# microsoft/hyperspace

Measured on AMD Instinct MI355X. Metric: index-build GB/s + indexed filter/join query latency (s), 1/2/4/8 MI355X, higher is better.
Workload: dtype int64/fp64 columnar; 1 GPU; model=covering-index(key,val) build + filter + co-bucketed join, num_buckets=200, parallelism=bucket-parallel dp1, RCCL all-to-all exchange, device=cuda

## Files before the change

### hyperspace_amd/csrc/binding.cpp

```cpp

#include <torch/extension.h>

#include <c10/hip/HIPStream.h>

#include <algorithm>
#include <string>
#include <tuple>
#include <vector>

#include "bucket_writer.h"
#include "kernels/kernels.h"

namespace {

hipStream_t current_stream() {
  return c10::hip::getCurrentHIPStream().stream();
}

void check_cuda(const torch::Tensor& t, const char* name) {
  TORCH_CHECK(t.is_cuda(), name, " must be a device tensor");
  TORCH_CHECK(t.is_contiguous(), name, " must be contiguous");
}

int normalize_dtype_code(torch::ScalarType t) {
// ... 500 lines not shown
                     ((uint32_t)d[pos + 3] << 24);
      pos += 4;
      TORCH_CHECK(pos + (int64_t)len <= end, "byte-array page ", p,
                  ": value overruns page");
      op[vi++] = (int32_t)written;
      memcpy(bp + written, d + pos, len);
      written += len;
      pos += len;
    }
  }
  op[vi] = (int32_t)written;
  return {offs, out.narrow(0, 0, written)};
}

void host_memcpy(torch::Tensor dst, int64_t off, py::buffer src) {
  TORCH_CHECK(!dst.is_cuda() && dst.scalar_type() == torch::kUInt8,
              "dst must be a cpu u8 tensor");
  py::buffer_info info = src.request();
  int64_t n = (int64_t)info.size * (int64_t)info.itemsize;
  TORCH_CHECK(off >= 0 && off + n <= dst.numel(),
              "host_memcpy out of range");
  uint8_t* d = dst.data_ptr<uint8_t>() + off;
  const void* s = info.ptr;
  {
    py::gil_scoped_release rel;
    memcpy(d, s, (size_t)n);
  }
}

std::vector<torch::Tensor> parse_rle_runs(torch::Tensor bytes,
                                           int64_t start, int64_t end,
                                           int64_t bit_width,
                                           int64_t num_values) {
  TORCH_CHECK(!bytes.is_cuda() && bytes.scalar_type() == torch::kUInt8,
              "bytes must be a cpu u8 tensor");
  const uint8_t* d = bytes.data_ptr<uint8_t>();
  std::vector<int64_t> kind, out_off, len, bitoff, value;
  int64_t pos = start, out = 0;
  int64_t bw_bytes = (bit_width + 7) / 8;
  while (out < num_values && pos < end) {
    uint64_t h = 0;
    int shift = 0;
    while (true) {
      TORCH_CHECK(pos < end, "rle: truncated varint");
      uint8_t b = d[pos++];
      h |= (uint64_t)(b & 0x7F) << shift;
      if (!(b & 0x80)) break;
      shift += 7;
    }
    if (h & 1) {
      int64_t groups = (int64_t)(h >> 1);
      int64_t count = groups * 8;
      if (count > num_values - out) count = num_values - out;
      kind.push_back(1);
      out_off.push_back(out);
      len.push_back(count);
      bitoff.push_back(pos * 8);
      value.push_back(0);
      pos += groups * bit_width;
      out += count;
    } else {
      int64_t run = (int64_t)(h >> 1);
      if (run > num_values - out) run = num_values - out;
      int64_t v = 0;
      for (int64_t i = 0; i < bw_bytes; i++) {
        TORCH_CHECK(pos < end, "rle: truncated repeat value");
        v |= (int64_t)d[pos++] << (8 * i);
      }
      kind.push_back(0);
      out_off.push_back(out);
      len.push_back(run);
      bitoff.push_back(0);
      value.push_back(v);
      out += run;
    }
  }
  TORCH_CHECK(out == num_values, "rle: produced ", out, " of ",
              num_values, " values");
  auto opts = torch::dtype(torch::kInt64);
  auto mk = [&](std::vector<int64_t>& v) {
    return torch::tensor(v, opts);
  };
  return {mk(kind), mk(out_off), mk(len), mk(bitoff), mk(value)};
}

torch::Tensor rle_decode(torch::Tensor src_u8_dev, torch::Tensor kind,
                         torch::Tensor out_off, torch::Tensor len,
                         torch::Tensor bitoff, torch::Tensor value,
                         int64_t bit_width, int64_t n_out) {
  check_cuda(src_u8_dev, "src");
  TORCH_CHECK(bit_width >= 0 && bit_width <= 32,
              "rle_decode: bit_width must be in 0..32, got ", bit_width);
  auto dev = src_u8_dev.device();
  auto k = kind.to(dev), o = out_off.to(dev), l = len.to(dev),
       b = bitoff.to(dev), v = value.to(dev);
  auto out = torch::empty({n_out},
                          torch::dtype(torch::kInt32).device(dev));
  hsk::rle_decode_indices(src_u8_dev.data_ptr<uint8_t>(),
                          k.data_ptr<int64_t>(), o.data_ptr<int64_t>(),
                          l.data_ptr<int64_t>(), b.data_ptr<int64_t>(),
                          v.data_ptr<int64_t>(), kind.numel(),
                          (int)bit_width,
                          (uint32_t*)out.data_ptr<int32_t>(), n_out,
                          current_stream());
  return out;
}

void copy_unaligned(torch::Tensor src_u8, int64_t src_off,
                    torch::Tensor dst, int64_t dst_byte_off,
                    int64_t nbytes) {
  TORCH_CHECK(src_u8.is_cuda() && dst.is_cuda(), "device tensors required");
  TORCH_CHECK(src_u8.scalar_type() == torch::kUInt8, "src must be u8");
  TORCH_CHECK(src_off + nbytes + 4 <= src_u8.numel(),
              "src buffer must extend 4 bytes past the payload");
  TORCH_CHECK(dst_byte_off % 4 == 0 && nbytes % 4 == 0, "4B granularity");
  hsk::copy_unaligned(src_u8.data_ptr<uint8_t>(), src_off,
                      (uint8_t*)dst.data_ptr(), dst_byte_off, nbytes,
                      current_stream());
}

torch::Tensor gather_rows(torch::Tensor values, torch::Tensor idx) {
  check_cuda(values, "values");
  check_cuda(idx, "idx");
  TORCH_CHECK(idx.scalar_type() == torch::kInt64 ||
                  idx.scalar_type() == torch::kInt32,
              "idx must be int64 or int32");
  auto out = torch::empty({idx.numel()}, values.options());
  if (idx.scalar_type() == torch::kInt32)
    hsk::gather(values.data_ptr(), idx.data_ptr<int32_t>(), out.data_ptr(),
                idx.numel(), (int)values.element_size(), current_stream());
  else
    hsk::gather(values.data_ptr(), idx.data_ptr<int64_t>(), out.data_ptr(),
                idx.numel(), (int)values.element_size(), current_stream());
  return out;
}

int bit_length_u64(uint64_t v) { return v ? 64 - __builtin_clzll(v) : 0; }

py::object bucket_sort_perm(torch::Tensor key, torch::Tensor bucket_ids,
                            int64_t num_buckets) {
  check_cuda(key, "key");
  check_cuda(bucket_ids, "bucket_ids");
  TORCH_CHECK(bucket_ids.scalar_type() == torch::kInt32,
              "bucket_ids must be int32");
  TORCH_CHECK(num_buckets > 0 && num_buckets <= (int64_t)INT32_MAX,
              "bucket_sort_perm: num_buckets must be in 1..INT32_MAX, got ",
              num_buckets);
  int dtype = normalize_dtype_code(key.scalar_type());
  TORCH_CHECK(dtype != 2 && dtype != 3,
              "bucket_sort_perm: integer keys only");
  int64_t n = key.numel();
  TORCH_CHECK(bucket_ids.numel() == n, "bucket_ids length mismatch");
  if (n <= 1 || n > (int64_t)INT32_MAX) return py::none();
  auto dev = key.device();
  auto i64 = torch::dtype(torch::kInt64).device(dev);
  auto i32 = torch::dtype(torch::kInt32).device(dev);
  auto stream = current_stream();

  auto mm = torch::empty({2}, i64);
  hsk::key_minmax(key.data_ptr(), dtype, n,
                  (uint64_t*)mm.data_ptr<int64_t>(), stream);
  auto mm_host = mm.cpu();
  uint64_t kmin = (uint64_t)mm_host.data_ptr<int64_t>()[0];
  uint64_t range = (uint64_t)mm_host.data_ptr<int64_t>()[1] - kmin;
  int bbits = bit_length_u64((uint64_t)num_buckets - 1);
  int kbits = bit_length_u64(range);
  if (kbits + bbits > 64) return py::none();
  int shift = (kbits + 7) / 8 * 8;
  if (shift + bbits > 64) shift = 64 - bbits;
  uint64_t low_mask = kbits ? ~0ull >> (64 - kbits) : 0;
  uint64_t mask = low_mask;
  if (bbits) mask |= (~0ull >> (64 - bbits)) << shift;

  auto comp = torch::empty({n}, i64);
  auto tmp_comp = torch::empty({n}, i64);
  auto perm = torch::empty({n}, i32);
  auto tmp_perm = torch::empty({n}, i32);
  auto hist = torch::empty({hsk::radix_sort_hist_size(n)}, i32);
  hsk::compose_bucket_key(key.data_ptr(), dtype,
                          bucket_ids.data_ptr<int32_t>(), kmin, shift,
                          (uint64_t*)comp.data_ptr<int64_t>(), n, stream);
  if (hsk::radix_sort_index32((uint64_t*)comp.data_ptr<int64_t>(),
                              perm.data_ptr<int32_t>(),
                              (uint64_t*)tmp_comp.data_ptr<int64_t>(),
                              tmp_perm.data_ptr<int32_t>(),
                              (uint32_t*)hist.data_ptr<int32_t>(), mask, n,
                              stream)) {
    std::swap(comp, tmp_comp);
    std::swap(perm, tmp_perm);
  }
  auto sorted = (const uint64_t*)comp.data_ptr<int64_t>();
  auto seg = torch::empty({num_buckets + 1}, i64);
  hsk::bucket_seg_offsets(sorted, n, shift, (int32_t)num_buckets,
                          seg.data_ptr<int64_t>(), stream);
  auto sorted_key = torch::empty_like(key);
  hsk::restore_key(sorted, low_mask, kmin, dtype, sorted_key.data_ptr(), n,
                   stream);
  return py::make_tuple(perm, sorted_key, seg.cpu());
}

torch::Tensor aligned16(torch::Tensor t) {
  if (t.numel() > 0 && reinterpret_cast<uintptr_t>(t.data_ptr()) % 16 != 0)
    return t.clone();
  return t;
}

torch::Tensor group_offsets(std::vector<torch::Tensor> keys,
                            std::vector<torch::Tensor> masks) {
  TORCH_CHECK(!keys.empty() && keys.size() <= 8, "1..8 key columns");
  TORCH_CHECK(masks.empty() || masks.size() == keys.size(),
              "masks must be empty or parallel to keys");
  int64_t n = keys[0].numel();
  auto dev = keys[0].device();
  auto opts = torch::dtype(torch::kInt64).device(dev);
  if (n == 0) return torch::zeros({1}, opts);
  std::vector<torch::Tensor> held;
  const uint64_t* kptr[8] = {nullptr};
  const uint8_t* mptr[8] = {nullptr};
  for (size_t c = 0; c < keys.size(); ++c) {
    check_cuda(keys[c], "key");
    TORCH_CHECK(keys[c].scalar_type() == torch::kInt64,
                "keys must be normalized int64");
    TORCH_CHECK(keys[c].numel() == n, "key column length mismatch");
    held.push_back(aligned16(keys[c]));
    kptr[c] = (const uint64_t*)held.back().data_ptr<int64_t>();
    if (!masks.empty() && masks[c].numel() > 0) {
      check_cuda(masks[c], "mask");
      TORCH_CHECK(masks[c].numel() == n, "mask length mismatch");
      TORCH_CHECK(masks[c].scalar_type() == torch::kBool ||
                      masks[c].scalar_type() == torch::kUInt8,
                  "mask must be bool/uint8");
      held.push_back(aligned16(masks[c]));
      mptr[c] = (const uint8_t*)held.back().data_ptr();
    }
  }
  auto stream = current_stream();
  int64_t tile = hsk::group_tile_size();
  int64_t n_tiles = (n + tile - 1) / tile;
  auto tile_counts = torch::empty({n_tiles}, opts);
  hsk::group_offsets_count(kptr, mptr, (int)keys.size(), n,
                           tile_counts.data_ptr<int64_t>(), stream);
  auto tile_offsets = torch::empty({n_tiles}, opts);
  auto total = torch::empty({1}, opts);
  hsk::exclusive_scan_i64(tile_counts.data_ptr<int64_t>(),
                          tile_offsets.data_ptr<int64_t>(), n_tiles,
                          total.data_ptr<int64_t>(), stream);
  int64_t n_groups = total.cpu().item<int64_t>();
  auto out = torch::empty({n_groups + 1}, opts);
  hsk::group_offsets_emit(kptr, mptr, (int)keys.size(), n,
                          tile_offsets.data_ptr<int64_t>(),
                          total.data_ptr<int64_t>(), out.data_ptr<int64_t>(),
                          stream);
  return out;
}

std::vector<torch::Tensor> segmented_reduce(torch::Tensor values,
                                            torch::Tensor valid,
                                            torch::Tensor offsets,
                                            int64_t want) {
  check_cuda(values, "values");
  int dtype;
  switch (values.scalar_type()) {
    case torch::kInt64: dtype = 0; break;
    case torch::kInt32: dtype = 1; break;
    case torch::kFloat64: dtype = 2; break;
    case torch::kFloat32: dtype = 3; break;
    default:
      TORCH_CHECK(false, "segmented_reduce: values must be int32, int64, "
                         "float32 or float64");
  }
  bool is_float = dtype >= 2;
  auto dev = values.device();
  int64_t n = values.numel();
  auto off_d = offsets.to(dev, torch::kInt64).contiguous();
  TORCH_CHECK(off_d.numel() >= 1, "offsets must have n_groups + 1 entries");
  int64_t n_groups = off_d.numel() - 1;
  auto i64 = torch::dtype(torch::kInt64).device(dev);
  auto sum_opts = is_float ? torch::dtype(torch::kFloat64).device(dev) : i64;
  auto sums = torch::zeros({(want & 1) ? n_groups : 0}, sum_opts);
  auto mins = torch::zeros({(want & 2) ? n_groups : 0}, values.options());
  auto maxs = torch::zeros({(want & 4) ? n_groups : 0}, values.options());
  auto counts = torch::zeros({n_groups}, i64);
  if (n == 0 || n_groups == 0) return {sums, mins, maxs, counts};
  values = aligned16(values);
  const uint8_t* vptr = nullptr;
  if (valid.numel() > 0) {
    check_cuda(valid, "valid");
    TORCH_CHECK(valid.numel() == n, "valid length mismatch");
    TORCH_CHECK(valid.scalar_type() == torch::kBool ||
                    valid.scalar_type() == torch::kUInt8,
                "valid must be bool/uint8");
    valid = aligned16(valid);
    vptr = (const uint8_t*)valid.data_ptr();
  }
  int64_t tile = hsk::group_tile_size();
  int64_t n_tiles = (n + tile - 1) / tile;
  auto tile_groups = torch::empty({n_tiles + 1}, i64);
  auto partials =
      torch::empty({4 * hsk::segmented_reduce_num_blocks(n)}, i64);
  hsk::segmented_reduce(values.data_ptr(), dtype, vptr,
                        off_d.data_ptr<int64_t>(), n, n_groups,
                        (want & 1) ? sums.data_ptr() : nullptr,
                        (want & 2) ? mins.data_ptr() : nullptr,
                        (want & 4) ? maxs.data_ptr() : nullptr,
                        counts.data_ptr<int64_t>(),
                        tile_groups.data_ptr<int64_t>(),
                        partials.data_ptr<int64_t>(), current_stream());
  return {sums, mins, maxs, counts};
}

int64_t group_tile_size() { return hsk::group_tile_size(); }

torch::Tensor topk_rows(torch::Tensor keys, int64_t k, torch::Tensor valid,
                        bool keep_ties) {
  check_cuda(keys, "keys");
  TORCH_CHECK(keys.scalar_type() == torch::kInt64,
              "keys must be normalized int64");
  int64_t n = keys.numel();
  auto opts = torch::dtype(torch::kInt64).device(keys.device());
  if (n == 0 || k <= 0) return torch::empty({0}, opts);
  if (k > n) k = n;
  keys = aligned16(keys);
  const uint8_t* vptr = nullptr;
  if (valid.numel() > 0) {
    check_cuda(valid, "valid");
    TORCH_CHECK(valid.numel() == n, "valid length mismatch");
    TORCH_CHECK(valid.scalar_type() == torch::kBool ||
                    valid.scalar_type() == torch::kUInt8,
                "valid must be bool/uint8");
    valid = aligned16(valid);
    vptr = (const uint8_t*)valid.data_ptr();
  }
  auto stream = current_stream();
  auto scratch = torch::zeros({hsk::topk_scratch_size(n)}, opts);
  const uint64_t* kp = (const uint64_t*)keys.data_ptr<int64_t>();
  int64_t* d_total = hsk::topk_select(kp, vptr, n, k, keep_ties,
                                      scratch.data_ptr<int64_t>(), stream);
  int64_t idx = d_total - scratch.data_ptr<int64_t>();
  int64_t n_out = scratch.narrow(0, idx, 1).cpu().item<int64_t>();
  TORCH_CHECK(n_out >= 0 && n_out <= n, "topk_rows: bad output length");
  auto out = torch::empty({n_out}, opts);
  hsk::topk_emit(kp, vptr, n, scratch.data_ptr<int64_t>(),
                 out.data_ptr<int64_t>(), n_out, stream);
  return out;
}

int64_t topk_tile_size() { return hsk::topk_tile_size(); }

std::tuple<std::vector<int64_t>, std::vector<int64_t>, std::vector<int64_t>,
           std::vector<int64_t>>
write_bucket_files(std::vector<torch::Tensor> cols,
// ... 195 lines not shown
```

### hyperspace_amd/execution/scan_stream.py

```python

from __future__ import annotations

from concurrent.futures import ThreadPoolExecutor
from typing import Iterator, List, Optional, Tuple

import torch

from .columnar import ColumnBatch
from ..config import IndexConstants


class ScanStream:
    def __init__(self, files, columns: List[str], device,
                 lineage_tracker=None, group_bytes: int = 1 << 30,
                 reader=None):
        self.files = list(files)
        self.columns = list(columns)
        self.device = device
        self.tracker = lineage_tracker
        self.group_bytes = max(1, group_bytes)
        self.reader = reader

    @property
    def total_bytes(self) -> int:
        return sum(f.size for f in self.files)

    def file_groups(self) -> List[List]:
        groups: List[List] = []
        cur: List = []
        cur_bytes = 0
        for f in self.files:
            if cur and cur_bytes + f.size > self.group_bytes:
                groups.append(cur)
                cur = []
                cur_bytes = 0
            cur.append(f)
            cur_bytes += f.size
        if cur:
            groups.append(cur)
        return groups

    def _load_group(self, group) -> ColumnBatch:
        paths = [f.name for f in group]
        if self.reader is not None:
            batch, row_counts = self.reader(paths, self.columns or None,
                                            self.device)
        else:
            from ..sources.parquet_io import (read_files_batch,
                                              read_files_batch_device)
            if self.device.type == "cuda":
                batch, row_counts = read_files_batch_device(
                    paths, self.device, columns=self.columns or None)
            else:
                batch, row_counts = read_files_batch(
                    paths, columns=self.columns or None)
        if self.tracker is not None:
            fids = torch.tensor(
                [self.tracker.add_file(f.name, f.size, f.modifiedTime)
                 for f in group], dtype=torch.int64, device=batch.device)
            counts = torch.tensor(row_counts, dtype=torch.int64,
                                  device=batch.device)
            batch = batch.with_column(
                IndexConstants.DATA_FILE_NAME_ID_COLUMN,
                torch.repeat_interleave(fids, counts))
        return batch

    def batches(self) -> Iterator[ColumnBatch]:
        groups = self.file_groups()
        if not groups:
            return
        with ThreadPoolExecutor(max_workers=1) as prefetcher:
            fut = prefetcher.submit(self._load_group, groups[0])
            for i in range(len(groups)):
                batch = fut.result()
                if i + 1 < len(groups):
                    fut = prefetcher.submit(self._load_group,
                                            groups[i + 1])
                yield batch

    def materialize(self) -> ColumnBatch:
        parts = list(self.batches())
        if not parts:
            from ..execution.executor import _empty_batch
            from ..log.entry import Schema, SchemaField
            return ColumnBatch({})
        if len(parts) == 1:
            return parts[0]
        return ColumnBatch.concat(parts)
```

### hyperspace_amd/index/covering/index.py

```python

from __future__ import annotations

import contextlib
import os
from typing import Any, Dict, List, Optional, Tuple

import torch

from ..base import Index, IndexerContext
from ...config import IndexConstants
from ...exceptions import HyperspaceException
from ...log.entry import (Schema, register_derived_dataset,
                          COVERING_INDEX_TYPE)
from ... import ops
from ...execution.columnar import ColumnBatch, StringColumn
from ...sources.parquet_io import (bucket_file_name, write_batch_parquet,
                                   read_files_batch, bucket_id_of_file)


class CoveringIndex(Index):
    def __init__(self, indexed_columns: List[str],
                 included_columns: List[str], schema: Schema,
                 num_buckets: int, properties: Dict[str, str]):
        self.indexed_columns = list(indexed_columns)
        self.included_columns = list(included_columns)
        self.schema = schema
        self.num_buckets = num_buckets
        self._properties = dict(properties)

    @property
    def kind(self) -> str:
        return "CoveringIndex"

    @property
    def kind_abbr(self) -> str:
        return "CI"

    def indexed_columns_list(self) -> List[str]:
        return list(self.indexed_columns)

    def referenced_columns(self) -> List[str]:
        return self.indexed_columns + self.included_columns

    @property
    def can_handle_deleted_files(self) -> bool:
        return (self._properties.get(IndexConstants.LINEAGE_PROPERTY, "false")
                .lower() == "true")

    @property
    def has_lineage(self) -> bool:
        return self.can_handle_deleted_files

    def with_new_properties(self, props: Dict[str, str]) -> "CoveringIndex":
        return CoveringIndex(self.indexed_columns, self.included_columns,
                             self.schema, self.num_buckets, props)

    def to_json(self) -> Dict[str, Any]:
        return {
            "type": COVERING_INDEX_TYPE,
            "indexedColumns": self.indexed_columns,
            "includedColumns": self.included_columns,
            "schema": self.schema.to_json(),
            "numBuckets": self.num_buckets,
            "properties": self._properties,
        }

    @staticmethod
    def from_json(d: Dict[str, Any]) -> "CoveringIndex":
        return CoveringIndex(
            d["indexedColumns"], d["includedColumns"],
            Schema.from_json(d["schema"]), d["numBuckets"],
            d.get("properties", {}))

    def write(self, ctx: IndexerContext, index_data) -> List[str]:
        from ...execution.scan_stream import ScanStream
        os.makedirs(ctx.index_data_path, exist_ok=True)

        import torch.distributed as dist
        distributed = dist.is_available() and dist.is_initialized() and \
            dist.get_world_size() > 1
        task_id = dist.get_rank() if distributed else 0

        if isinstance(index_data, ScanStream):
            batches = index_data.batches()
            n_groups = len(index_data.file_groups())
        else:
            batches = iter([index_data])
            n_groups = 1

        if distributed:
            from ...parallel import dist_context as dc
            t = dc.collective_tensor([n_groups])
            dist.all_reduce(t, op=dist.ReduceOp.MAX)
            n_groups = int(t[0])
            written = self._write_distributed(ctx, batches, n_groups,
                                              task_id)
        else:
            written = []
            for g in range(n_groups):
                try:
                    batch = next(batches)
                except StopIteration:
                    batch = self._empty_batch(ctx)
                written.extend(self._write_group(ctx, batch, task_id))
        if n_groups > 1:
            ctx.built_for_cache = None
        return written

    def _bucket_ids(self, batch: ColumnBatch) -> torch.Tensor:
        from ...ops.string_hash import bucket_hash_keys
        keys = bucket_hash_keys(batch, self.indexed_columns)
        key_masks = [batch.mask(c) for c in self.indexed_columns]
        return ops.murmur3_bucket(
            keys, self.num_buckets,
            key_masks if any(m is not None for m in key_masks) else None)

    def _write_distributed(self, ctx, batches, n_groups: int,
                           task_id: int) -> List[str]:
        import torch.distributed as dist
        from ...parallel import dist_context as dc
        from ...parallel.exchange import BucketExchange
        n = self.num_buckets
        ex = BucketExchange(n)
        ctx.exchange_stats = ex
        chunk_bytes = int(ctx.session.conf.get(
            "spark.hyperspace.exchange.chunkBytes", 1 << 30))
        written: List[str] = []
        recv_acc: Dict[int, list] = {}

        def flush_group(g: int) -> None:
            parts = recv_acc.pop(g, [])
            parts = [(b, k) for b, k in parts if b.num_rows]
            if not parts:
                return
            if len(parts) == 1:
                rb, rbk = parts[0]
            else:
                rb = ColumnBatch.concat([p[0] for p in parts])
                rbk = torch.cat([p[1] for p in parts])
            batch, seg = sort_by_bucket_and_keys(
                rb, rbk, self.indexed_columns, n)
            out = write_bucketed(batch, seg, ctx.index_data_path, n,
                                 task_id)
            ctx.built_for_cache = (batch, seg, list(out))
            written.extend(out)

        prev = None
        for g in range(n_groups):
            try:
                batch = next(batches)
            except StopIteration:
                batch = self._empty_batch(ctx)
            local_chunks = 1
            if chunk_bytes > 0 and batch.num_rows:
                local_chunks = max(
                    1, -(-batch.nbytes() // chunk_bytes))
            t = dc.collective_tensor([local_chunks])
            dist.all_reduce(t, op=dist.ReduceOp.MAX)
            nchunks = int(t[0])
            rows = batch.num_rows
            for c in range(nchunks):
                lo = rows * c // nchunks
                hi = rows * (c + 1) // nchunks
                sub = batch.slice(lo, hi) if nchunks > 1 else batch
                pend = ex.start(sub, self._bucket_ids(sub))
                if prev is not None:
                    p, pg, plast = prev
                    recv_acc.setdefault(pg, []).append(ex.finish(p))
                    if plast:
                        flush_group(pg)
                prev = (pend, g, c == nchunks - 1)
        if prev is not None:
            p, pg, _ = prev
            recv_acc.setdefault(pg, []).append(ex.finish(p))
            flush_group(pg)
        return written

    def _write_group(self, ctx, batch: ColumnBatch,
                     task_id: int) -> List[str]:
        import time as _time
        timing = os.environ.get("HS_TIMING")
        n = self.num_buckets
        t0 = _time.perf_counter()
        bucket_ids = self._bucket_ids(batch)
        if batch.num_rows == 0:
            return []
        t1 = _time.perf_counter()

        pipeline = (batch.device.type == "cuda" and n >= 8
                    and batch.num_rows >= 1 << 22
                    and bool(os.environ.get("HS_PIPE_WRITE")))
        if not pipeline:
            batch, seg = sort_by_bucket_and_keys(
                batch, bucket_ids, self.indexed_columns, n)
            if timing:
                import torch as _torch
                if batch.device.type == "cuda":
                    _torch.cuda.synchronize()
            t2 = _time.perf_counter()
            out = write_bucketed(batch, seg, ctx.index_data_path, n,
                                 task_id)
            ctx.built_for_cache = (batch, seg, list(out))
            if timing:
                import sys as _sys
                print(f"[hs-timing] build group: hash {t1-t0:.3f}s "
                      f"sort {t2-t1:.3f}s write "
                      f"{_time.perf_counter()-t2:.3f}s",
                      file=_sys.stderr)
            return out

        import torch as _torch
        from concurrent.futures import ThreadPoolExecutor
        b64 = bucket_ids.to(_torch.int64)
        perm = ops.sort_perm(ops.normalize_key(b64))
        batch = batch.gather(perm)
        sorted_b = ops.gather_rows(b64, perm)
        seg = _bucket_seg_offsets(sorted_b, n)
        t2 = _time.perf_counter()

        nb_batches = min(8, n)
        bounds = [round(i * n / nb_batches) for i in range(nb_batches + 1)]
        pool = ThreadPoolExecutor(max_workers=2)
        futures = []
        pieces: List[ColumnBatch] = []
        for i in range(nb_batches):
            b_lo, b_hi = bounds[i], bounds[i + 1]
            r_lo, r_hi = int(seg[b_lo]), int(seg[b_hi])
            if r_hi <= r_lo:
                continue
            sub = batch.slice(r_lo, r_hi)
            sub_sorted, lseg = sort_by_bucket_and_keys(
                sub, sorted_b[r_lo:r_hi], self.indexed_columns, n)
            ev = _torch.cuda.Event()
            ev.record()
            pieces.append(sub_sorted)
            futures.append(pool.submit(
                write_bucketed, sub_sorted, lseg, ctx.index_data_path,
                n, task_id, ev))
        out = []
        for f in futures:
            out.extend(f.result())
        pool.shutdown()
        if timing:
            _torch.cuda.synchronize()
        t3 = _time.perf_counter()
        full = (ColumnBatch.concat(pieces) if len(pieces) > 1
                else pieces[0]) if pieces else batch
        ctx.built_for_cache = (full, seg, list(out))
        if timing:
            import sys as _sys
            print(f"[hs-timing] build group: hash {t1-t0:.3f}s "
                  f"partition {t2-t1:.3f}s sort+write(pipe) "
                  f"{t3-t2:.3f}s", file=_sys.stderr)
        return out

    def _empty_batch(self, ctx) -> ColumnBatch:
        import torch as _torch
        dts = {"long": _torch.int64, "integer": _torch.int32,
               "short": _torch.int16, "byte": _torch.int8,
               "date": _torch.int32,
               "double": _torch.float64, "float": _torch.float32,
               "boolean": _torch.bool}
        cols: Dict[str, Any] = {}
        for f in self.schema.fields:
            if f.type == "string":
                cols[f.name] = StringColumn(
                    _torch.empty(0, dtype=_torch.int32,
                                 device=ctx.session.device), [])
            else:
                cols[f.name] = _torch.empty(
                    0, dtype=dts.get(f.type, _torch.int64),
                    device=ctx.session.device)
        return ColumnBatch(cols)

    def optimize(self, ctx: IndexerContext,
                 files_to_optimize: List[str]) -> List[str]:
        os.makedirs(ctx.index_data_path, exist_ok=True)
        by_bucket: Dict[int, List[str]] = {}
        for p in files_to_optimize:
            b = bucket_id_of_file(p)
            if b is None:
                raise HyperspaceException(f"Not a bucketed index file: {p}")
            by_bucket.setdefault(b, []).append(p)
        from concurrent.futures import ThreadPoolExecutor

        def compact_one(item):
            b, paths = item
            sub, _ = read_files_batch(sorted(paths))
            if ctx.session.device.type == "cuda":
                sub = sub.to(ctx.session.device)
            perm = _multi_key_sort_perm(sub, self.indexed_columns)
            sub = sub.gather(perm)
            out = os.path.join(ctx.index_data_path, bucket_file_name(0, b))
            write_batch_parquet(sub.to("cpu") if sub.device.type == "cuda"
                                else sub, out)
            return out

        items = sorted(by_bucket.items())
        if len(items) <= 2:
            return [compact_one(i) for i in items]
        with ThreadPoolExecutor(max_workers=8) as pool:
            return list(pool.map(compact_one, items))

    def refresh_incremental(self, ctx: IndexerContext,
                            appended_batch: Optional[ColumnBatch],
                            deleted_file_ids: List[int],
                            previous_files: List[str]
                            ) -> Tuple[List[str], List[str]]:
        written: List[str] = []
        if appended_batch is not None and appended_batch.num_rows:
            written.extend(self.write(ctx, appended_batch))
        kept = list(previous_files)
        if deleted_file_ids:
            if not self.has_lineage:
                raise HyperspaceException(
                    "Index has no lineage column; cannot handle deletes")
            os.makedirs(ctx.index_data_path, exist_ok=True)
            ids = torch.tensor(sorted(deleted_file_ids), dtype=torch.int64)
            kept = []
            lineage_col = IndexConstants.DATA_FILE_NAME_ID_COLUMN
            for p in previous_files:
                b = bucket_id_of_file(p)
                sub, _ = read_files_batch([p])
                lineage = sub.tensor(lineage_col)
                keep_mask = ~ops.isin_sorted(lineage, ids)
                if bool(keep_mask.all()):
                    kept.append(p)
                    continue
                sub = sub.gather(
                    torch.nonzero(keep_mask, as_tuple=False).flatten())
                if sub.num_rows == 0:
                    continue
                out = os.path.join(ctx.index_data_path,
                                   bucket_file_name(1, b or 0))
                write_batch_parquet(sub, out)
                written.append(out)
        return written, kept

    def statistics(self) -> Dict[str, Any]:
        return {"indexedColumns": self.indexed_columns,
                "includedColumns": self.included_columns,
                "numBuckets": self.num_buckets}



def _multi_key_sort_perm(batch: ColumnBatch, key_cols: List[str]
                         ) -> torch.Tensor:
    n = batch.num_rows
    dev = batch.device
    perm = torch.arange(n, dtype=torch.int64, device=dev)
    for c in reversed(key_cols):
        keys = ops.sql_key(batch.tensor(c))[perm]
        _, perm = ops.sort_pairs(keys, perm)
        m = batch.mask(c)
        if m is not None and not bool(m.all()):
            f = m[perm]
            perm = perm[torch.cat([
                torch.nonzero(~f, as_tuple=False).flatten(),
                torch.nonzero(f, as_tuple=False).flatten()])]
    return perm


def _bucket_seg_offsets(sorted_bkeys_u64: torch.Tensor, num_buckets: int
                        ) -> torch.Tensor:
    probes = ops.cpu_ref.normalize_key(
        torch.arange(num_buckets + 1, dtype=torch.int64)).to(
            sorted_bkeys_u64.device)
    if sorted_bkeys_u64.numel() and int(sorted_bkeys_u64.max()) >= 0 \
            and int(sorted_bkeys_u64.min()) >= 0:
        seg = torch.searchsorted(
            sorted_bkeys_u64,
            torch.arange(num_buckets + 1, dtype=torch.int64,
                         device=sorted_bkeys_u64.device))
        return seg.cpu()
    sortable = sorted_bkeys_u64 ^ (-0x8000000000000000)
    sortable_probes = probes ^ (-0x8000000000000000)
    return torch.searchsorted(sortable, sortable_probes).cpu()


def _fused_bucket_sort(batch: ColumnBatch, bucket_ids: torch.Tensor,
                       key_cols: List[str], num_buckets: int
                       ) -> Optional[Tuple[ColumnBatch, torch.Tensor]]:
    if len(key_cols) != 1 or os.environ.get("HS_FUSED_BUCKET_SORT") == "0":
        return None
    key_name = batch._stored_key(key_cols[0])
    key = batch.columns[key_name]
    if isinstance(key, StringColumn) or batch.has_nulls(key_name):
        return None
    res = ops.bucket_sort_perm(key, bucket_ids, num_buckets)
    if res is None:
        return None
    perm, sorted_key, seg = res
    cols: Dict[str, Any] = {}
    for k, v in batch.columns.items():
        if k == key_name:
            cols[k] = sorted_key
        elif isinstance(v, StringColumn):
            cols[k] = StringColumn(ops.gather_rows(v.codes, perm), v.values)
        else:
            cols[k] = ops.gather_rows(v, perm)
    return ColumnBatch(
        cols, {k: m[perm] for k, m in batch.masks.items()}), seg


def sort_by_bucket_and_keys(batch: ColumnBatch, bucket_ids: torch.Tensor,
                            key_cols: List[str], num_buckets: int
                            ) -> Tuple[ColumnBatch, torch.Tensor]:
    fused = _fused_bucket_sort(batch, bucket_ids, key_cols, num_buckets)
    if fused is not None:
        return fused
    perm = _multi_key_sort_perm(batch, key_cols)
    b64 = ops.gather_rows(bucket_ids.to(torch.int64), perm)
    sorted_bkeys, perm2 = ops.sort_pairs(ops.normalize_key(b64), perm)
    batch = batch.gather(perm2)
    probes = ops.cpu_ref.normalize_key(
        torch.arange(num_buckets + 1, dtype=torch.int64)).to(
            sorted_bkeys.device)
    sortable = sorted_bkeys ^ (-0x8000000000000000)
    sortable_probes = probes ^ (-0x8000000000000000)
    seg = torch.searchsorted(sortable, sortable_probes).cpu()
    return batch, seg


_NATIVE_WRITE_DTYPES = (torch.int64, torch.int32, torch.float64,
                        torch.float32)
_WRITE_RING_SLOTS = 64


def _native_write_eligible(batch: ColumnBatch) -> bool:
    if os.environ.get("HS_NATIVE_WRITE") == "0" or batch.masks:
        return False
    if not batch.columns or not ops.native.available():
        return False
    return all(not isinstance(c, StringColumn)
               and c.dtype in _NATIVE_WRITE_DTYPES and c.dim() == 1
               and c.device == batch.device
               for c in batch.columns.values())


def _device_stat_unusable(v) -> bool:
    return v != v or v == 0


def _bucket_statistics(batch: ColumnBatch, jobs) -> Tuple[list, list]:
    from ...sources.native_parquet import _statistics
    ncols = len(batch.columns)
    mins = [b""] * (len(jobs) * ncols)
    maxs = [b""] * (len(jobs) * ncols)
    on_device = batch.device.type == "cuda"
    offsets = torch.tensor([jobs[0][1]] + [j[2] for j in jobs],
                           dtype=torch.int64)
    for c, col in enumerate(batch.columns.values()):
        mm = None
        if on_device:
            lo0, hi1 = jobs[0][1], jobs[-1][2]
            red = ops.segmented_reduce(col[lo0:hi1], None, offsets - lo0,
                                       want=("min", "max"))
            mm = torch.stack([red["min"], red["max"]]).cpu().numpy()
        for f, (_, lo, hi, _) in enumerate(jobs):
            if mm is not None and not (
                    col.dtype.is_floating_point
                    and (_device_stat_unusable(mm[0, f])
                         or _device_stat_unusable(mm[1, f]))):
                mn, mx = mm[0, f].tobytes(), mm[1, f].tobytes()
            else:
                mn, mx = _statistics(col[lo:hi].cpu().numpy())
            mins[f * ncols + c] = mn
            maxs[f * ncols + c] = mx
    return mins, maxs


def _write_bucketed_native(batch: ColumnBatch, jobs,
                           after_event: Optional["torch.cuda.Event"]
                           ) -> List[str]:
    import time as _time
    import numpy as np
    from ...sources.native_parquet import (ColumnChunkLayout, Page,
                                           _layout_cache_put)
    from ...sources.staging import _pinned_get, _pinned_put
    timing = os.environ.get("HS_TIMING")
    t0 = _time.perf_counter()
    on_device = batch.device.type == "cuda"
    names = list(batch.columns.keys())
    cols = [c.contiguous() for c in batch.columns.values()]
    chunk = max(1, int(float(os.environ.get("HS_WRITE_CHUNK_MB", "8"))
                       * (1 << 20)))
    threads = min(15, max(1, int(os.environ.get("HS_WRITE_THREADS", "15"))))
    paths = [j[3] for j in jobs]
    row_lo = [j[1] for j in jobs]
    row_hi = [j[2] for j in jobs]
    ring = None
    streams = (0, 0)
    if on_device:
        if after_event is not None:
            torch.cuda.current_stream(batch.device).wait_event(after_event)
        esz = max(c.element_size() for c in cols)
        largest = max(hi - lo for lo, hi in zip(row_lo, row_hi)) * esz
        chunk = min(chunk, -(-largest // 4096) * 4096)
        n_chunks = sum(-(-(hi - lo) * c.element_size() // chunk)
                       for lo, hi in zip(row_lo, row_hi) for c in cols)
        ring = _pinned_get(chunk * max(2, min(_WRITE_RING_SLOTS, n_chunks)))
    try:
        with torch.cuda.device(batch.device) if on_device \
                else contextlib.nullcontext():
            mins, maxs = _bucket_statistics(batch, jobs)
            t1 = _time.perf_counter()
            if on_device:
                pool = [torch.cuda.Stream(device=batch.device)
                        for _ in range(2)]
                streams = tuple(s.cuda_stream for s in pool)
            sizes, mtimes, starts, ends = ops.native.ext().write_bucket_files(
                cols, names, paths, row_lo, row_hi, mins, maxs,
                ring if ring is not None
                else torch.empty(0, dtype=torch.uint8),
                chunk, threads, streams[0], streams[1], bool(timing))
    finally:
        if ring is not None:
            _pinned_put(ring)
    ncols = len(cols)
    np_dtypes = [np.dtype(str(c.dtype).replace("torch.", "")) for c in cols]
    for f, path in enumerate(paths):
        rows = row_hi[f] - row_lo[f]
        _layout_cache_put(path, rows, [
            ColumnChunkLayout(
                names[c], np_dtypes[c],
                [Page("plain", starts[f * ncols + c], ends[f * ncols + c],
                      rows)], rows, "plain", None, [None])
            for c in range(ncols)], (sizes[f], mtimes[f]))
    if timing:
        import sys as _sys
# ... 68 lines not shown
```

### hyperspace_amd/sources/parquet_io.py

```python

from __future__ import annotations

import itertools
import os
import re
import sys
import threading
import time
import uuid
from concurrent.futures import ThreadPoolExecutor, as_completed
from typing import Dict, List, NamedTuple, Optional, Tuple

import numpy as np
import torch

from ..exceptions import HyperspaceException
from .device_decode import (DecodeState, convert_logical, decode_chunks,
                            split_row_groups)
from .logical_types import (Conv, check_parquet_file, parquet_convs,
                            to_storage_np)
from .native_parquet import (StrCol, layout_cache_get, merge_string_dicts,
                             read_native_layout, string_remap_tables)
from .staging import _DEV_RATIO, _pinned_get, _pinned_put

# ... 95 lines not shown
    if native_ok and paths:
        names = list(per_file[0].keys())
        if columns is not None:
            order = {c.lower(): i for i, c in enumerate(columns)}
            names.sort(key=lambda n: order.get(n.lower(), 99))
        from ..execution.columnar import StringColumn
        merged = {}
        merged_masks = {}
        for name in names:
            arrs = [f[name] for f in per_file]
            if any(isinstance(a, StrCol) for a in arrs):
                dicts = [a.values for a in arrs]
                mvals, remap = merge_string_dicts(dicts)
                parts = [a.codes for a in arrs]
                if remap:
                    parts = [part if lut is None
                             else np.array(lut, dtype=np.int32)[part]
                             for part, lut in zip(
                                 parts, string_remap_tables(mvals, dicts))]
                codes = np.concatenate(parts) if len(parts) > 1 else parts[0]
                merged[name] = StringColumn(
                    torch.from_numpy(np.ascontiguousarray(codes)),
                    list(mvals))
            else:
                merged[name] = torch.from_numpy(
                    np.concatenate(arrs) if len(arrs) > 1 else arrs[0])
            if any(name in fm for fm in per_file_masks):
                mparts = [fm.get(name, np.ones(rc, dtype=bool))
                          for fm, rc in zip(per_file_masks, row_counts)]
                merged_masks[name] = torch.from_numpy(
                    np.concatenate(mparts) if len(mparts) > 1
                    else mparts[0])
        return ColumnBatch(merged, merged_masks), row_counts

    import pyarrow.parquet as pq
    import pyarrow as pa
    tables = []
    row_counts = []
    for p in paths:
        check_parquet_file(p, columns)
        t = pq.read_table(p, columns=_resolve_read_columns(p, columns))
        tables.append(t)
        row_counts.append(t.num_rows)
    if not tables:
        return ColumnBatch({}), []
    table = pa.concat_tables(tables, promote_options="default")
    batch = ColumnBatch.from_arrow(table)
    if columns is not None:
        batch = batch.select(columns)
    return batch, row_counts


_PHYS_TO_NP = {"INT64": np.dtype("int64"), "INT32": np.dtype("int32"),
               "DOUBLE": np.dtype("float64"), "FLOAT": np.dtype("float32")}
_NP_TO_TORCH = {np.dtype("int64"): torch.int64,
                np.dtype("int32"): torch.int32,
                np.dtype("float64"): torch.float64,
                np.dtype("float32"): torch.float32}
_N_STREAMS = 16


class _ReadPlan(NamedTuple):
    names: List[str]
    dtypes: Dict[str, np.dtype]
    convs: Dict[str, Conv]
    row_counts: List[int]
    nullable_cols: set
    string_cols: set
    layouts: Optional[list]
    metas: list
    schemas: list


def _plan_from_cache(cached, want) -> _ReadPlan:
    lay0 = cached[0][1]
    return _ReadPlan(
        [c.name for c in lay0 if want is None or c.name.lower() in want],
        {c.name: c.np_dtype for c in lay0},
        {c.name: c.conv for c in lay0 if c.conv is not None},
        [ent[0] for ent in cached],
        {c.name for ent in cached for c in ent[1] if c.has_nulls},
        {c.name for ent in cached for c in ent[1] if c.is_string},
        [[c for c in ent[1] if want is None or c.name.lower() in want]
         for ent in cached], [], [])


def _plan_from_footers(paths, want) -> Optional[_ReadPlan]:
    import pyarrow.parquet as pq
    metas = []
    schemas = []
    for p in paths:
        try:
            pf = pq.ParquetFile(p)
        except Exception:
            return None
        metas.append(pf.metadata)
        schemas.append(pf.schema)
    file_convs = [parquet_convs(sch, want) for sch in schemas]
    nullable_cols = set()
    for md, sch in zip(metas, schemas):
        for rg_i in range(md.num_row_groups):
            rg = md.row_group(rg_i)
            for ci in range(rg.num_columns):
                col = rg.column(ci)
                st = col.statistics
                if st is None or st.null_count is None:
                    if sch.column(ci).max_definition_level > 0:
                        return None
                elif st.null_count > 0:
                    nullable_cols.add(col.path_in_schema)
    rg0 = metas[0].row_group(0)
    names = []
    dtypes = {}
    convs = {}
    string_cols = set()
    for ci in range(rg0.num_columns):
        col = rg0.column(ci)
        name = col.path_in_schema
        if want is not None and name.lower() not in want:
            continue
        npd = _PHYS_TO_NP.get(col.physical_type)
        if npd is None:
            sch_col = schemas[0].column(ci)
            if col.physical_type == "BYTE_ARRAY":
                npd = np.dtype("int32")
                string_cols.add(name)
            elif col.physical_type == "FIXED_LEN_BYTE_ARRAY" and \
                    sch_col.logical_type.type == "DECIMAL" and \
                    sch_col.precision <= 18:
                npd = np.dtype("int64")
            elif col.physical_type == "INT96":
                npd = np.dtype("int64")
            else:
                return None
        names.append(name)
        dtypes[name] = npd
        if ci in file_convs[0]:
            convs[name] = file_convs[0][ci]
    return _ReadPlan(names, dtypes, convs, [md.num_rows for md in metas],
                     nullable_cols, string_cols, None, metas, schemas)


def _plan_device_read(paths, columns) -> Optional[_ReadPlan]:
    want = {c.lower() for c in columns} if columns is not None else None
    cached = [layout_cache_get(p) for p in paths]
    plan = (_plan_from_cache(cached, want) if None not in cached
            else _plan_from_footers(paths, want))
    if plan is not None and columns is not None:
        order = {c.lower(): i for i, c in enumerate(columns)}
        plan.names.sort(key=lambda n: order.get(n.lower(), 99))
    return plan


class _DeviceRead:

    def __init__(self, paths, columns, device, plan: _ReadPlan):
        from ..ops import native as native_ext
        self.paths, self.columns, self.plan = paths, columns, plan
        total_rows = int(sum(plan.row_counts))
        self.st = DecodeState(
            device, native_ext.ext(), plan.names,
            np.concatenate([[0], np.cumsum(plan.row_counts)[:-1]]),
            {n: torch.empty(total_rows, dtype=_NP_TO_TORCH[plan.dtypes[n]],
                            device=device) for n in plan.names},
            {n: torch.ones(total_rows, dtype=torch.bool, device=device)
             for n in plan.names if n in plan.nullable_cols},
            os.environ.get("HS_DECODE_TIMING"))
        self.streams = [torch.cuda.Stream(device=device)
                        for _ in range(_N_STREAMS)]
        self.infos: List[Optional[tuple]] = [None] * len(paths)
        self.dev_bufs: List[Optional[torch.Tensor]] = [None] * len(paths)
        self.upload_events: list = [None] * len(paths)
        self.upload_lock = threading.Lock()
        self.uids = itertools.count()

    def load_file(self, i):
        p = self.paths[i]
        size = os.path.getsize(p)
        buf = _pinned_get(size + 4)
        view = memoryview(buf.numpy())
        with open(p, "rb", buffering=0) as f:
            f.readinto(view[:size])
        if self.plan.layouts is not None:
            return buf, size, self.plan.layouts[i]
        lay = read_native_layout(p, self.columns, data=view[:size],
                                 meta=self.plan.metas[i],
                                 pf_schema=self.plan.schemas[i])
        if lay is None:
            _pinned_put(buf)
            return None, 0, None
        return buf, size, lay[1]

    def host_unit(self, i):
        st, plan = self.st, self.plan
        cols, fmasks, n = _pyarrow_file_dict(self.paths[i], self.columns)
        assert n == plan.row_counts[i], (self.paths[i], n,
                                         plan.row_counts[i])
        low = {k.lower(): v for k, v in cols.items()}
        mlow = {k.lower(): v for k, v in fmasks.items()}
        base = int(st.file_base[i])
        with torch.cuda.stream(self.streams[i % _N_STREAMS]):
            for name in plan.names:
                arr = low[name.lower()]
                if isinstance(arr, StrCol):
                    st.str_chunks.append((name, base, base + n,
                                          arr.values))
                    arr = arr.codes
                else:
                    arr = to_storage_np(arr, plan.dtypes[name])
                st.out[name][base:base + n] = torch.from_numpy(
                    np.ascontiguousarray(arr)).to(st.device,
                                                  non_blocking=True)
                m = mlow.get(name.lower())
                if name in st.out_masks and m is not None:
                    st.out_masks[name][base:base + n] = \
                        torch.from_numpy(m).to(st.device, non_blocking=True)

    def decode_unit(self, uid, i, row_off, chunks):
        buf, size, _ = self.infos[i]
        t0 = time.perf_counter()
        stream = self.streams[uid % _N_STREAMS]
        with torch.cuda.stream(stream):
            with self.upload_lock:
                if self.dev_bufs[i] is None:
                    self.dev_bufs[i] = buf[:size + 4].to(
                        self.st.device, non_blocking=True)
                    self.upload_events[i] = torch.cuda.Event()
                    self.upload_events[i].record(stream)
                else:
                    stream.wait_event(self.upload_events[i])
            decode_chunks(self.st, i, buf, self.dev_bufs[i], chunks, row_off)
        if self.st.timing == "2":
            print(f"[hs-unit] u{uid} rows={chunks[0].num_values} chunks="
                  f"{[(c.name, c.encoding, len(c.pages)) for c in chunks]} "
                  f"{time.perf_counter()-t0:.3f}s", file=sys.stderr)

    def units(self, i):
        chunks = self.infos[i][2]
        if chunks is None:
            return [(self.host_unit, i)]
        groups = (split_row_groups(chunks) if len(self.paths) < _N_STREAMS
                  else [(0, chunks)])
        return [(self.decode_unit, next(self.uids), i, row_off, rg_chunks)
                for row_off, rg_chunks in groups]

    def run(self) -> int:
        n_units = 0
        workers = int(os.environ.get("HS_DECODE_WORKERS", "16"))
        if len(self.paths) > 2 and workers > 1:
            dec_futs = []
            with ThreadPoolExecutor(max_workers=16) as read_pool, \
                    ThreadPoolExecutor(max_workers=workers) as dec_pool:
                read_futs = {read_pool.submit(self.load_file, i): i
                             for i in range(len(self.paths))}
                for fut in as_completed(read_futs):
                    i = read_futs[fut]
                    self.infos[i] = fut.result()
                    dec_futs += [dec_pool.submit(*u) for u in self.units(i)]
                for f in dec_futs:
                    f.result()
            return len(dec_futs)
        for i in range(len(self.paths)):
            self.infos[i] = self.load_file(i)
        for i in range(len(self.paths)):
            for fn, *args in self.units(i):
                fn(*args)
                n_units += 1
        return n_units


def _merge_string_columns(st: DecodeState, string_cols) -> None:
    from ..execution.columnar import StringColumn
    by_name: Dict[str, list] = {}
    for name, lo, hi, vals in st.str_chunks:
        by_name.setdefault(name, []).append((lo, hi, vals))
    for name in string_cols:
        runs = by_name.get(name, [])
        dicts = [v for _, _, v in runs]
        merged, remap = merge_string_dicts(dicts)
        if not dicts:
            merged = [""]
        if remap:
            tables = string_remap_tables(merged, dicts)
            for (lo, hi, _), lut in zip(runs, tables):
                if lut is not None:
                    lut = torch.tensor(lut, dtype=torch.int32,
                                       device=st.device)
                    st.out[name][lo:hi] = lut[st.out[name][lo:hi].long()]
        st.out[name] = StringColumn(st.out[name], list(merged))


def read_files_batch_device(paths: List[str], device,
                            columns: Optional[List[str]] = None):
    from ..execution.columnar import ColumnBatch

    def fallback():
        batch, rc = read_files_batch(paths, columns)
        return batch.to(device), rc

    plan = _plan_device_read(paths, columns)
    if plan is None:
        return fallback()
    rd = _DeviceRead(paths, columns, device, plan)
    st = rd.st
    t1 = time.perf_counter()
    n_units = rd.run()
    t2 = time.perf_counter()
    cur = torch.cuda.current_stream()
    for s in rd.streams:
        cur.wait_stream(s)
    cur.synchronize()
    if st.timing:
        print(f"[hs-decode] files={len(paths)} units={n_units} "
              f"read+decode(pipe) {t2-t1:.3f}s "
              f"sync {time.perf_counter()-t2:.3f}s", file=sys.stderr)
    snappy_bad = bool(torch.cat(st.statuses).ne(0).any().item()) \
        if st.statuses else False
    for b in [inf[0] for inf in rd.infos] + st.keepalive:
        if b is not None:
            _pinned_put(b)
    if snappy_bad:
        return fallback()
    if plan.string_cols:
        _merge_string_columns(st, plan.string_cols)
    for name, conv in plan.convs.items():
        st.out[name] = convert_logical(st.out[name], conv)
    return ColumnBatch(st.out, st.out_masks), plan.row_counts
```

Measured before the change: 17.31 GB/s.

## Pipeline index build: sort keys on side stream while other columns decode

Adds a column-phased parquet read that reads and decodes the key column first, then runs the fused bucket sort on a separate stream while the remaining columns are still being read and decoded. The other columns are then gathered by the resulting permutation before the bucketed write. The native bucket_sort_perm now releases the GIL so Python decode threads can progress during its host syncs, and the old env-gated HS_PIPE_WRITE path is removed. This adds a second read path with fallbacks (ColumnReadRefused) and per-file device buffers that raise peak memory.

Result: slower. 15.82 GB/s (-8.6%).

```diff
diff --git a/hyperspace_amd/csrc/binding.cpp b/hyperspace_amd/csrc/binding.cpp
--- a/hyperspace_amd/csrc/binding.cpp
+++ b/hyperspace_amd/csrc/binding.cpp
@@ -676,6 +676,9 @@
   int64_t n = key.numel();
   TORCH_CHECK(bucket_ids.numel() == n, "bucket_ids length mismatch");
   if (n <= 1 || n > (int64_t)INT32_MAX) return py::none();
+  torch::Tensor perm, sorted_key, seg_host;
+  {
+  py::gil_scoped_release no_gil;
   auto dev = key.device();
   auto i64 = torch::dtype(torch::kInt64).device(dev);
   auto i32 = torch::dtype(torch::kInt32).device(dev);
@@ -689,7 +692,10 @@
   uint64_t range = (uint64_t)mm_host.data_ptr<int64_t>()[1] - kmin;
   int bbits = bit_length_u64((uint64_t)num_buckets - 1);
   int kbits = bit_length_u64(range);
-  if (kbits + bbits > 64) return py::none();
+  if (kbits + bbits > 64) {
+    py::gil_scoped_acquire gil;
+    return py::none();
+  }
   int shift = (kbits + 7) / 8 * 8;
   if (shift + bbits > 64) shift = 64 - bbits;
   uint64_t low_mask = kbits ? ~0ull >> (64 - kbits) : 0;
@@ -698,7 +704,7 @@
 
   auto comp = torch::empty({n}, i64);
   auto tmp_comp = torch::empty({n}, i64);
-  auto perm = torch::empty({n}, i32);
+  perm = torch::empty({n}, i32);
   auto tmp_perm = torch::empty({n}, i32);
   auto hist = torch::empty({hsk::radix_sort_hist_size(n)}, i32);
   hsk::compose_bucket_key(key.data_ptr(), dtype,
@@ -717,10 +723,12 @@
   auto seg = torch::empty({num_buckets + 1}, i64);
   hsk::bucket_seg_offsets(sorted, n, shift, (int32_t)num_buckets,
                           seg.data_ptr<int64_t>(), stream);
-  auto sorted_key = torch::empty_like(key);
+  sorted_key = torch::empty_like(key);
   hsk::restore_key(sorted, low_mask, kmin, dtype, sorted_key.data_ptr(), n,
                    stream);
-  return py::make_tuple(perm, sorted_key, seg.cpu());
+  seg_host = seg.cpu();
+  }
+  return py::make_tuple(perm, sorted_key, seg_host);
 }
 
 torch::Tensor aligned16(torch::Tensor t) {
diff --git a/hyperspace_amd/execution/scan_stream.py b/hyperspace_amd/execution/scan_stream.py
--- a/hyperspace_amd/execution/scan_stream.py
+++ b/hyperspace_amd/execution/scan_stream.py
@@ -39,6 +39,18 @@
         if cur:
             groups.append(cur)
         return groups
+
+    def reads_plain_parquet(self) -> bool:
+        if self.tracker is not None:
+            return False
+        if self.reader is None:
+            return True
+        from ..sources.parquet_source import ParquetRelation
+        rel = getattr(self.reader, "__self__", None)
+        return (type(rel) is ParquetRelation
+                and getattr(self.reader, "__func__", None)
+                is ParquetRelation.read_files
+                and not rel.partition_schema().fields)
 
     def _load_group(self, group) -> ColumnBatch:
         paths = [f.name for f in group]
diff --git a/hyperspace_amd/index/covering/index.py b/hyperspace_amd/index/covering/index.py
--- a/hyperspace_amd/index/covering/index.py
+++ b/hyperspace_amd/index/covering/index.py
@@ -80,6 +80,16 @@
         distributed = dist.is_available() and dist.is_initialized() and \
             dist.get_world_size() > 1
         task_id = dist.get_rank() if distributed else 0
+
+        if isinstance(index_data, ScanStream) and not distributed:
+            from . import pipelined_build as pb
+            plan = pb.plan_pipelined_build(self, ctx, index_data)
+            if plan is not None:
+                try:
+                    return pb.pipelined_build(self, ctx, index_data, plan,
+                                              task_id)
+                except pb.ColumnReadRefused:
+                    pass
 
         if isinstance(index_data, ScanStream):
             batches = index_data.batches()
@@ -187,71 +197,21 @@
             return []
         t1 = _time.perf_counter()
 
-        pipeline = (batch.device.type == "cuda" and n >= 8
-                    and batch.num_rows >= 1 << 22
-                    and bool(os.environ.get("HS_PIPE_WRITE")))
-        if not pipeline:
-            batch, seg = sort_by_bucket_and_keys(
-                batch, bucket_ids, self.indexed_columns, n)
-            if timing:
-                import torch as _torch
-                if batch.device.type == "cuda":
-                    _torch.cuda.synchronize()
-            t2 = _time.perf_counter()
-            out = write_bucketed(batch, seg, ctx.index_data_path, n,
-                                 task_id)
-            ctx.built_for_cache = (batch, seg, list(out))
-            if timing:
-                import sys as _sys
-                print(f"[hs-timing] build group: hash {t1-t0:.3f}s "
-                      f"sort {t2-t1:.3f}s write "
-                      f"{_time.perf_counter()-t2:.3f}s",
-                      file=_sys.stderr)
-            return out
-
-        import torch as _torch
-        from concurrent.futures import ThreadPoolExecutor
-        b64 = bucket_ids.to(_torch.int64)
-        perm = ops.sort_perm(ops.normalize_key(b64))
-        batch = batch.gather(perm)
-        sorted_b = ops.gather_rows(b64, perm)
-        seg = _bucket_seg_offsets(sorted_b, n)
+        batch, seg = sort_by_bucket_and_keys(
+            batch, bucket_ids, self.indexed_columns, n)
+        if timing:
+            import torch as _torch
+            if batch.device.type == "cuda":
+                _torch.cuda.synchronize()
         t2 = _time.perf_counter()
-
-        nb_batches = min(8, n)
-        bounds = [round(i * n / nb_batches) for i in range(nb_batches + 1)]
-        pool = ThreadPoolExecutor(max_workers=2)
-        futures = []
-        pieces: List[ColumnBatch] = []
-        for i in range(nb_batches):
-            b_lo, b_hi = bounds[i], bounds[i + 1]
-            r_lo, r_hi = int(seg[b_lo]), int(seg[b_hi])
-            if r_hi <= r_lo:
-                continue
-            sub = batch.slice(r_lo, r_hi)
-            sub_sorted, lseg = sort_by_bucket_and_keys(
-                sub, sorted_b[r_lo:r_hi], self.indexed_columns, n)
-            ev = _torch.cuda.Event()
-            ev.record()
-            pieces.append(sub_sorted)
-            futures.append(pool.submit(
-                write_bucketed, sub_sorted, lseg, ctx.index_data_path,
-                n, task_id, ev))
-        out = []
-        for f in futures:
-            out.extend(f.result())
-        pool.shutdown()
-        if timing:
-            _torch.cuda.synchronize()
-        t3 = _time.perf_counter()
-        full = (ColumnBatch.concat(pieces) if len(pieces) > 1
-                else pieces[0]) if pieces else batch
-        ctx.built_for_cache = (full, seg, list(out))
+        out = write_bucketed(batch, seg, ctx.index_data_path, n, task_id)
+        ctx.built_for_cache = (batch, seg, list(out))
         if timing:
             import sys as _sys
             print(f"[hs-timing] build group: hash {t1-t0:.3f}s "
-                  f"partition {t2-t1:.3f}s sort+write(pipe) "
-                  f"{t3-t2:.3f}s", file=_sys.stderr)
+                  f"sort {t2-t1:.3f}s write "
+                  f"{_time.perf_counter()-t2:.3f}s",
+                  file=_sys.stderr)
         return out
 
     def _empty_batch(self, ctx) -> ColumnBatch:
@@ -359,23 +319,6 @@
                 torch.nonzero(~f, as_tuple=False).flatten(),
                 torch.nonzero(f, as_tuple=False).flatten()])]
     return perm
-
-
-def _bucket_seg_offsets(sorted_bkeys_u64: torch.Tensor, num_buckets: int
-                        ) -> torch.Tensor:
-    probes = ops.cpu_ref.normalize_key(
-        torch.arange(num_buckets + 1, dtype=torch.int64)).to(
-            sorted_bkeys_u64.device)
-    if sorted_bkeys_u64.numel() and int(sorted_bkeys_u64.max()) >= 0 \
-            and int(sorted_bkeys_u64.min()) >= 0:
-        seg = torch.searchsorted(
-            sorted_bkeys_u64,
-            torch.arange(num_buckets + 1, dtype=torch.int64,
-                         device=sorted_bkeys_u64.device))
-        return seg.cpu()
-    sortable = sorted_bkeys_u64 ^ (-0x8000000000000000)
-    sortable_probes = probes ^ (-0x8000000000000000)
-    return torch.searchsorted(sortable, sortable_probes).cpu()
 
 
 def _fused_bucket_sort(batch: ColumnBatch, bucket_ids: torch.Tensor,
diff --git a/hyperspace_amd/index/covering/pipelined_build.py b/hyperspace_amd/index/covering/pipelined_build.py
--- /dev/null
+++ b/hyperspace_amd/index/covering/pipelined_build.py
@@ -0,0 +1,121 @@
+
+from __future__ import annotations
+
+import os
+import sys
+import time
+from typing import Dict, List, Optional
+
+import numpy as np
+import torch
+
+from ... import ops
+from ...execution.columnar import ColumnBatch
+from ...sources.parquet_io import (ColumnPhasedRead, ColumnReadRefused,
+                                   plan_column_read)
+
+_DEFAULT_MIN_ROWS = 1 << 22
+_KEY_DTYPES = (np.dtype("int64"), np.dtype("int32"))
+_sort_streams: Dict[int, "torch.cuda.Stream"] = {}
+
+
+def _sort_stream(device) -> "torch.cuda.Stream":
+    idx = device.index if device.index is not None \
+        else torch.cuda.current_device()
+    if idx not in _sort_streams:
+        _sort_streams[idx] = torch.cuda.Stream(device=device)
+    return _sort_streams[idx]
+
+
+def _key_name(index, plan) -> Optional[str]:
+    want = index.indexed_columns[0].lower()
+    return next((nm for nm in plan.names if nm.lower() == want), None)
+
+
+def plan_pipelined_build(index, ctx, stream):
+    if os.environ.get("HS_PIPE_BUILD") == "0" \
+            or os.environ.get("HS_FUSED_BUCKET_SORT") == "0":
+        return None
+    dev = stream.device
+    if getattr(dev, "type", "cpu") != "cuda" or not ops.native.available():
+        return None
+    if len(index.indexed_columns) != 1 or not stream.columns:
+        return None
+    if not stream.reads_plain_parquet():
+        return None
+    groups = stream.file_groups()
+    if len(groups) != 1:
+        return None
+    plan = plan_column_read([f.name for f in groups[0]], stream.columns)
+    if plan is None:
+        return None
+    key = _key_name(index, plan)
+    if key is None or plan.dtypes[key] not in _KEY_DTYPES:
+        return None
+    rows = int(sum(plan.row_counts))
+    min_rows = int(os.environ.get("HS_PIPE_BUILD_MIN_ROWS",
+                                  _DEFAULT_MIN_ROWS))
+    if rows < max(2, min_rows) or rows >= 1 << 31:
+        return None
+    return plan
+
+
+def pipelined_build(index, ctx, stream, plan, task_id: int) -> List[str]:
+    from .index import write_bucketed
+    timing = os.environ.get("HS_TIMING")
+    dev = stream.device
+    n = index.num_buckets
+    paths = [f.name for f in stream.file_groups()[0]]
+    key = _key_name(index, plan)
+    others = [nm for nm in plan.names if nm != key]
+    t0 = time.perf_counter()
+    with torch.cuda.device(dev):
+        sort_stream = _sort_stream(dev)
+        rd = ColumnPhasedRead(paths, dev, plan)
+        marks = []
+        sort = []
+
+        def mark(s):
+            if timing:
+                ev = torch.cuda.Event(enable_timing=True)
+                ev.record(s)
+                marks.append(ev)
+
+        mark(torch.cuda.current_stream())
+
+        def column_hook(name, events):
+            if name != key:
+                return
+            with torch.cuda.stream(sort_stream):
+                for ev in events:
+                    sort_stream.wait_event(ev)
+                mark(sort_stream)
+                kcol = rd.columns[key]
+                bucket_ids = index._bucket_ids(ColumnBatch({key: kcol}))
+                res = ops.bucket_sort_perm(kcol, bucket_ids, n)
+                mark(sort_stream)
+            if res is not None:
+                sort.append(res)
+
+        decoded, _ = rd.run([key] + others, column_hook)
+        sort_stream.synchronize()
+        if not sort:
+            return index._write_group(ctx, decoded, task_id)
+        perm, sorted_key, seg = sort[0]
+        batch = ColumnBatch({
+            nm: (sorted_key if nm == key
+                 else ops.gather_rows(decoded.columns[nm], perm))
+            for nm in plan.names})
+        del decoded, rd, perm, sort
+        if timing:
+            torch.cuda.synchronize()
+        t_read = time.perf_counter()
+        out = write_bucketed(batch, seg, ctx.index_data_path, n, task_id)
+        ctx.built_for_cache = (batch, seg, list(out))
+        if timing:
+            print(f"[hs-timing] pipelined build: keys decoded "
+                  f"{marks[0].elapsed_time(marks[1]) / 1e3:.3f}s sort done "
+                  f"{marks[0].elapsed_time(marks[2]) / 1e3:.3f}s read+gather "
+                  f"done {t_read - t0:.3f}s write done "
+                  f"{time.perf_counter() - t0:.3f}s", file=sys.stderr)
+        return out
diff --git a/hyperspace_amd/sources/parquet_io.py b/hyperspace_amd/sources/parquet_io.py
--- a/hyperspace_amd/sources/parquet_io.py
+++ b/hyperspace_amd/sources/parquet_io.py
@@ -271,6 +271,101 @@
     return plan
 
 
+class ColumnReadRefused(Exception):
+    """A file turned out not to be readable column by column after the
+    plan accepted it (a page walk that fails, a truncated file).  Nothing
+    final has been produced: the caller reads the batch the usual way."""
+
+
+def _layout_byte_range(c) -> Tuple[int, int]:
+    spans = [(p.start, p.end) for p in c.pages]
+    if c.dict_page is not None:
+        spans.append((c.dict_page.start, c.dict_page.end))
+    return min(s for s, _ in spans), max(e for _, e in spans)
+
+
+def _footer_byte_ranges(md, name: str, size: int) -> List[Tuple[int, int]]:
+    ranges = []
+    for rg_i in range(md.num_row_groups):
+        rg = md.row_group(rg_i)
+        for ci in range(rg.num_columns):
+            col = rg.column(ci)
+            if col.path_in_schema != name:
+                continue
+            start = col.data_page_offset
+            if col.has_dictionary_page and \
+                    0 < col.dictionary_page_offset < start:
+                start = col.dictionary_page_offset
+            end = start + col.total_compressed_size
+            if not 0 <= start <= end <= size:
+                raise ColumnReadRefused(
+                    f"column {name}: chunk [{start}, {end}) outside the "
+                    f"file's {size} bytes")
+            ranges.append((start, end))
+    return ranges
+
+
+def plan_column_read(paths, columns) -> Optional[_ReadPlan]:
+    try:
+        plan = _plan_device_read(paths, columns)
+    except HyperspaceException:
+        return None
+    if plan is None or not plan.names or plan.nullable_cols \
+            or plan.string_cols or plan.convs:
+        return None
+    if plan.layouts is not None:
+        ok = all(c.codec == "UNCOMPRESSED" and not c.is_string
+                 and not c.has_nulls and c.conv is None
+                 and c.encoding in ("plain", "dict")
+                 for lay in plan.layouts for c in lay)
+        return plan if ok else None
+    want = set(plan.names)
+    for md in plan.metas:
+        if md.num_row_groups == 0:
+            return None
+        for rg_i in range(md.num_row_groups):
+            rg = md.row_group(rg_i)
+            seen = set()
+            for ci in range(rg.num_columns):
+                col = rg.column(ci)
+                if col.path_in_schema not in want:
+                    continue
+                seen.add(col.path_in_schema)
+                if col.compression.upper() != "UNCOMPRESSED" \
+                        or _PHYS_TO_NP.get(col.physical_type) \
+                        != plan.dtypes[col.path_in_schema]:
+                    return None
+            if seen != want:
+                return None
+    return plan
+
+
+class ColumnPhasedRead:
+
+    def __init__(self, paths: List[str], device, plan: _ReadPlan):
+        self._rd = _DeviceRead(paths, list(plan.names), device, plan)
+        self.plan = plan
+        self.columns = self._rd.st.out
+
+    def run(self, column_order: List[str], column_hook=None):
+        from ..execution.columnar import ColumnBatch
+        assert sorted(column_order) == sorted(self.plan.names), \
+            (column_order, self.plan.names)
+        rd = self._rd
+        try:
+            rd.run_columns(column_order, column_hook)
+        finally:
+            cur = torch.cuda.current_stream()
+            for s in rd.streams:
+                cur.wait_stream(s)
+            cur.synchronize()
+            for inf in rd.infos:
+                if inf is not None and inf[0] is not None:
+                    _pinned_put(inf[0])
+        return (ColumnBatch(rd.st.out, rd.st.out_masks),
+                self.plan.row_counts)
+
+
 class _DeviceRead:
 
     def __init__(self, paths, columns, device, plan: _ReadPlan):
@@ -292,6 +387,8 @@
         self.upload_events: list = [None] * len(paths)
         self.upload_lock = threading.Lock()
         self.uids = itertools.count()
+        self._tl = threading.local()
+        self._stream_ids = itertools.count()
 
     def load_file(self, i):
         p = self.paths[i]
@@ -362,6 +459,84 @@
                   else [(0, chunks)])
         return [(self.decode_unit, next(self.uids), i, row_off, rg_chunks)
                 for row_off, rg_chunks in groups]
+
+    def _file_buffers(self, i):
+        if self.infos[i] is None:
+            size = os.path.getsize(self.paths[i])
+            self.infos[i] = (_pinned_get(size + 4), size, None)
+            self.dev_bufs[i] = torch.empty(
+                size + 4, dtype=torch.uint8, device=self.st.device)
+        return self.infos[i][0], self.infos[i][1], self.dev_bufs[i]
+
+    def _column_chunks(self, i, name, view, size):
+        cached = self.plan.layouts is not None
+        if cached:
+            chunks = [c for c in self.plan.layouts[i] if c.name == name]
+            ranges = [_layout_byte_range(c) for c in chunks]
+        else:
+            ranges = _footer_byte_ranges(self.plan.metas[i], name, size)
+        fd = os.open(self.paths[i], os.O_RDONLY)
+        try:
+            for a, b in ranges:
+                while a < b:
+                    got = os.preadv(fd, [view[a:b]], a)
+                    if got <= 0:
+                        raise ColumnReadRefused(
+                            f"{self.paths[i]}: short read at {a}")
+                    a += got
+        finally:
+            os.close(fd)
+        if not cached:
+            lay = read_native_layout(self.paths[i], [name], data=view[:size],
+                                     meta=self.plan.metas[i],
+                                     pf_schema=self.plan.schemas[i])
+            if lay is None or not lay[1]:
+                raise ColumnReadRefused(
+                    f"{self.paths[i]}: column {name} has no native layout")
+            chunks = lay[1]
+        return ranges, chunks
+
+    def column_unit(self, name, i):
+        tl = self._tl
+        if not hasattr(tl, "stream"):
+            tl.stream = self.streams[next(self._stream_ids) % _N_STREAMS]
+            tl.last = None
+        stream = tl.stream
+        with torch.cuda.stream(stream):
+            buf, size, dev = self._file_buffers(i)
+            ranges, chunks = self._column_chunks(
+                i, name, memoryview(buf.numpy()), size)
+            if tl.last is not None:
+                tl.last.synchronize()
+            for a, b in ranges:
+                dev[a:b].copy_(buf[a:b], non_blocking=True)
+            decode_chunks(self.st, i, buf, dev, chunks, 0)
+            ev = torch.cuda.Event()
+            ev.record(stream)
+            tl.last = ev
+        return ev
+
+    def run_columns(self, order, column_hook=None) -> None:
+        workers = int(os.environ.get("HS_DECODE_WORKERS", "16"))
+        files = range(len(self.paths))
+        for i in files:
+            self._file_buffers(i)
+        if len(self.paths) <= 2 or workers <= 1:
+            for name in order:
+                events = [self.column_unit(name, i) for i in files]
+                if column_hook is not None:
+                    column_hook(name, events)
+            return
+        pool = ThreadPoolExecutor(max_workers=min(16, workers))
+        try:
+            futs = [[pool.submit(self.column_unit, name, i) for i in files]
+                    for name in order]
+            for name, col_futs in zip(order, futs):
+                events = [f.result() for f in col_futs]
+                if column_hook is not None:
+                    column_hook(name, events)
+        finally:
+            pool.shutdown(wait=True, cancel_futures=True)
 
     def run(self) -> int:
         n_units = 0
```
